# achao2013/deep3dmap

Hardware: AMD Instinct MI355X
Metric: rendered Mpix/s fwd+bwd, 100k-tri mesh @512x512 (higher is better)
Workload: dtype f32

## Files before the change

### deep3dmap_amd/csrc/d3m_forward.h

```cpp
#pragma once
#include "d3m_device.h"

namespace d3m {

struct BinBuffers {
    int B, F, S, tiles_x, tiles_y, T, kcap;
    void* rect;
    int* tile_count;
    int* tile_cursor;
    int* big_count;
    int* alloc_cursor;
    int* tile_offset;
    int* big_list;
    int* pairs;
};

constexpr uint32_t RECT_NONE = 0xFFFFFFFFu;
struct TileRect { int tx0, ty0, w, h; bool none, big; };
struct Rect64 {
    typedef uint2 T;
    static __device__ __forceinline__ T pack(int tx0, int ty0, int tx1, int ty1, bool big) {
        (void)big;
        return make_uint2((uint32_t)tx0 | ((uint32_t)ty0 << 16), (uint32_t)tx1 | ((uint32_t)ty1 << 16));
    }
    static __device__ __forceinline__ T none() { return make_uint2(RECT_NONE, 0); }
    static __device__ __forceinline__ TileRect unpack(T r, int kcap) {
        TileRect t;
        t.none = r.x == RECT_NONE;
        t.tx0 = r.x & 0xFFFF; t.ty0 = r.x >> 16;
        t.w = (int)(r.y & 0xFFFF) - t.tx0 + 1; t.h = (int)(r.y >> 16) - t.ty0 + 1;
        t.big = !t.none && t.w * t.h > kcap;
        return t;
    }
};
struct Rect32 {
    typedef uint32_t T;
    static constexpr uint32_t BIG = 0xFFFFFFFEu;
    static __device__ __forceinline__ T pack(int tx0, int ty0, int tx1, int ty1, bool big) {
        if (big) return BIG;
        return (uint32_t)tx0 | ((uint32_t)ty0 << 10) | ((uint32_t)(tx1 - tx0) << 20) | ((uint32_t)(ty1 - ty0) << 26);
    }
    static __device__ __forceinline__ T none() { return RECT_NONE; }
    static __device__ __forceinline__ TileRect unpack(T r, int kcap) {
        (void)kcap;
        TileRect t;
        t.none = r == RECT_NONE; t.big = r == BIG;
        t.tx0 = r & 0x3FF; t.ty0 = (r >> 10) & 0x3FF; t.w = (int)((r >> 20) & 0x3F) + 1; t.h = (int)(r >> 26) + 1;
        return t;
    }
};

__device__ __forceinline__ bool pixel_bbox(const float* f, int S, int& x0, int& x1, int& y0, int& y1) {
    if (f[0] == f[3] && f[3] == f[6] && f[1] == f[4] && f[4] == f[7]) return false;
    const bool finite = __builtin_isfinite(f[0]) && __builtin_isfinite(f[1]) && __builtin_isfinite(f[3]) &&
                        __builtin_isfinite(f[4]) && __builtin_isfinite(f[6]) && __builtin_isfinite(f[7]);
    if (!finite) {
        x0 = 0; y0 = 0; x1 = S - 1; y1 = S - 1;
        return true;
    }
    const float xmn = fminf(f[0], fminf(f[3], f[6])), xmx = fmaxf(f[0], fmaxf(f[3], f[6]));
    const float ymn = fminf(f[1], fminf(f[4], f[7])), ymx = fmaxf(f[1], fmaxf(f[4], f[7]));
    const double m = 4e-6 * ((double)fmaxf(fmaxf(fabsf(xmn), fabsf(xmx)), fmaxf(fabsf(ymn), fabsf(ymx))) + 1.0);
    const double lx = ceil((((double)xmn - m) * S + S - 1) * 0.5), hx = floor((((double)xmx + m) * S + S - 1) * 0.5);
    const double ly = ceil((((double)ymn - m) * S + S - 1) * 0.5), hy = floor((((double)ymx + m) * S + S - 1) * 0.5);
    if (lx > S - 1 || hx < 0 || ly > S - 1 || hy < 0 || lx > hx || ly > hy) return false;
    x0 = d2i(fmax(lx, 0.0));
    y0 = d2i(fmax(ly, 0.0));
    x1 = d2i(fmin(hx, (double)(S - 1)));
    y1 = d2i(fmin(hy, (double)(S - 1)));
    return true;
}

#ifndef D3M_BIN_THREADS
#define D3M_BIN_THREADS 1024
#endif
constexpr int BIN_THREADS = D3M_BIN_THREADS;
constexpr int BIN_THREADS_SMALL = 256;
constexpr int TA_BITS = BIN_THREADS >= 1024 ? 11 : BIN_THREADS >= 512 ? 10 : 9;
constexpr int TA_SLOTS = 1 << TA_BITS;
constexpr int TA_PROBES = 12;
constexpr int BIN_TABLE_TILES = 4;
__device__ __forceinline__ int ta_bits() { return blockDim.x >= 1024 ? TA_BITS : blockDim.x >= 512 ? TA_BITS - 1 : TA_BITS - 2; }
struct TileAgg {
    int key[TA_SLOTS];
    int cnt[TA_SLOTS];
    int base[TA_SLOTS];
};

__device__ __forceinline__ void ta_clear(TileAgg& t) {
    for (int k = threadIdx.x; k < (1 << ta_bits()); k += blockDim.x) { t.key[k] = 0; t.cnt[k] = 0; }
    __syncthreads();
}

__device__ __forceinline__ int ta_add(TileAgg& t, int tile, int& rank) {
    const int bits = ta_bits();
    unsigned h = ((unsigned)tile * 2654435761u) >> (32 - bits);
    for (int p = 0; p < TA_PROBES; p++, h = (h + 1) & ((1u << bits) - 1)) {
        int k = t.key[h];
        if (k == 0) k = atomicCAS(&t.key[h], 0, tile + 1);
        if (k == 0 || k == tile + 1) {
            rank = atomicAdd(&t.cnt[h], 1);
            return (int)h;
        }
    }
    return -1;
}

template <class FS, bool PAIRED, class RECT>
__global__ void __launch_bounds__(BIN_THREADS) k_bin_count(FS fs, BinBuffers bb, float* __restrict__ faces_inv,
                                                  float* __restrict__ faces_dense_out,
                                                  unsigned char* __restrict__ marks = nullptr,
                                                  int* __restrict__ marks_count = nullptr) {
    __shared__ TileAgg agg;
    if (marks_count && blockIdx.x == 0 && threadIdx.x == 0) *marks_count = 0;
    ta_clear(agg);
    const int F = bb.F, Fl = PAIRED ? F / 2 : F;
    const long lane_i = (long)blockIdx.x * blockDim.x + threadIdx.x;
    const bool in_range = lane_i < (long)bb.B * Fl;
    const int b = in_range ? (int)(lane_i / Fl) : 0, f0 = in_range ? (int)(lane_i % Fl) : 0;
    float loaded[9] = {0, 0, 0, 0, 0, 0, 0, 0, 0};
    if (in_range) fs.load(b, f0, loaded);
#pragma unroll
    for (int side = 0; side < (PAIRED ? 2 : 1); side++) {
        const int f = f0 + side * Fl;
        const long i = (long)b * F + f;
        float face[9];
#pragma unroll
        for (int k = 0; k < 9; k++) face[k] = side == 0 ? loaded[k] : loaded[(2 - k / 3) * 3 + k % 3];
        typename RECT::T r = RECT::none();
        int tx0 = 0, tx1 = -1, ty0 = 0, ty1 = -1;
        bool small = false;
        if (in_range) {
            if (!backside(face)) {
                if (faces_inv) {
                    float fi[9];
                    face_inverse(face, bb.S, fi);
#pragma unroll
                    for (int k = 0; k < 9; k++) faces_inv[i * 9 + k] = fi[k];
                }
                int x0, x1, y0, y1;
                if (pixel_bbox(face, bb.S, x0, x1, y0, y1)) {
                    if (faces_dense_out) {
#pragma unroll
                        for (int k = 0; k < 9; k++) faces_dense_out[i * 9 + k] = face[k];
                    }
                    tx0 = x0 / TILE_W; tx1 = x1 / TILE_W; ty0 = y0 / TILE_H; ty1 = y1 / TILE_H;
                    small = (tx1 - tx0 + 1) * (ty1 - ty0 + 1) <= bb.kcap;
                    r = RECT::pack(tx0, ty0, tx1, ty1, !small);
                    if (!small) {
                        const int pos = atomicAdd(&bb.big_count[b], 1);
                        bb.big_list[(size_t)b * F + pos] = f;
                    }
                }
            }
            reinterpret_cast<typename RECT::T*>(bb.rect)[i] = r;
            if (marks) marks[i] = 0;
        }
        const int w = small ? tx1 - tx0 + 1 : 0, nt = small ? w * (ty1 - ty0 + 1) : 0;
        for (int s = 0; s < nt; s++) {
            const int tile = b * bb.T + (ty0 + s / w) * bb.tiles_x + tx0 + s % w;
            int rank;
            if (s >= BIN_TABLE_TILES || ta_add(agg, tile, rank) < 0) atomicAdd(&bb.tile_count[tile], 1);
        }
    }
    __syncthreads();
    for (int k = threadIdx.x; k < (1 << ta_bits()); k += blockDim.x)
        if (agg.key[k]) atomicAdd(&bb.tile_count[agg.key[k] - 1], agg.cnt[k]);
}

constexpr int BIN_ALLOC_THREADS = 1024;
__global__ void __launch_bounds__(BIN_ALLOC_THREADS) k_bin_alloc(BinBuffers bb) {
    __shared__ int s_wave[BIN_ALLOC_THREADS / 64];
    __shared__ int s_base;
    const int n = bb.B * bb.T;
    const int i = blockIdx.x * BIN_ALLOC_THREADS + threadIdx.x;
    const int c = i < n ? bb.tile_count[i] : 0;
    const int incl = wave_inclusive_scan(c);
    const int lane = lane_id(), wv = threadIdx.x >> 6;
    if (lane == 63) s_wave[wv] = incl;
    __syncthreads();
    if (threadIdx.x == 0) {
        int run = 0;
        for (int k = 0; k < BIN_ALLOC_THREADS / 64; k++) { const int tk = s_wave[k]; s_wave[k] = run; run += tk; }
        s_base = atomicAdd(bb.alloc_cursor, run);
    }
    __syncthreads();
    if (i < n) bb.tile_offset[i] = s_base + s_wave[wv] + incl - c;
}

template <bool PAIRED, int FPT, class RECT>
__global__ void __launch_bounds__(BIN_THREADS) k_bin_fill(BinBuffers bb) {
    const typename RECT::T* __restrict__ rects = reinterpret_cast<const typename RECT::T*>(bb.rect);
    __shared__ TileAgg agg;
    ta_clear(agg);
    const int Fl = PAIRED ? bb.F / 2 : bb.F;
    constexpr int TA_LOCAL = BIN_TABLE_TILES;
    int packed[FPT][TA_LOCAL], face_of[FPT];
#pragma unroll
    for (int it = 0; it < FPT; it++) {
        const long lane_i = ((long)blockIdx.x * FPT + it) * blockDim.x + threadIdx.x;
        int tx0 = 0, ty0 = 0, w = 0, nt = 0, b = 0, f = 0;
        if (lane_i < (long)bb.B * Fl) {
            b = (int)(lane_i / Fl);
            const int f0 = (int)(lane_i % Fl);
            TileRect r = RECT::unpack(rects[(size_t)b * bb.F + f0], bb.kcap);
            f = f0;
            if (PAIRED) {
                const TileRect r1 = RECT::unpack(rects[(size_t)b * bb.F + f0 + Fl], bb.kcap);
                if (r.none) { r = r1; f = f0 + Fl; }
                else if (!r1.none && !r1.big) {
                    const int an = r1.w * r1.h;
                    for (int s2 = 0; s2 < an; s2++) {
                        const int tile = b * bb.T + (r1.ty0 + s2 / r1.w) * bb.tiles_x + r1.tx0 + s2 % r1.w;
                        const int pos = atomicAdd(&bb.tile_cursor[tile], 1);
                        bb.pairs[(size_t)bb.tile_offset[tile] + pos] = f0 + Fl;
                    }
                }
            }
            if (!r.none && !r.big) {
                tx0 = r.tx0; ty0 = r.ty0;
                w = r.w;
                nt = w * r.h;
            }
        }
        face_of[it] = f;
#pragma unroll
        for (int s = 0; s < TA_LOCAL; s++) packed[it][s] = -1;
        for (int s = 0; s < nt && s < TA_LOCAL; s++) {
            const int tile = b * bb.T + (ty0 + s / w) * bb.tiles_x + tx0 + s % w;
            int rank = 0;
            const int slot = ta_add(agg, tile, rank);
            if (slot >= 0) {
#pragma unroll
                for (int q = 0; q < TA_LOCAL; q++) if (q == s) packed[it][q] = (slot << 16) | rank;
            } else {
                const int pos = atomicAdd(&bb.tile_cursor[tile], 1);
                bb.pairs[(size_t)bb.tile_offset[tile] + pos] = f;
            }
        }
        for (int s0 = TA_LOCAL; s0 < nt; s0 += 4) {
            int tile[4], pos[4], off[4];
#pragma unroll
            for (int j = 0; j < 4; j++) {
                const int s = min(s0 + j, nt - 1);
                tile[j] = b * bb.T + (ty0 + s / w) * bb.tiles_x + tx0 + s % w;
            }
#pragma unroll
            for (int j = 0; j < 4; j++) {
                if (s0 + j < nt) { pos[j] = atomicAdd(&bb.tile_cursor[tile[j]], 1); off[j] = bb.tile_offset[tile[j]]; }
            }
#pragma unroll
            for (int j = 0; j < 4; j++)
                if (s0 + j < nt) bb.pairs[(size_t)off[j] + pos[j]] = f;
        }
    }
    __syncthreads();
    for (int k = threadIdx.x; k < (1 << ta_bits()); k += blockDim.x)
        if (agg.key[k]) {
            const int tile = agg.key[k] - 1;
            agg.base[k] = bb.tile_offset[tile] + atomicAdd(&bb.tile_cursor[tile], agg.cnt[k]);
        }
    __syncthreads();
#pragma unroll
    for (int it = 0; it < FPT; it++) {
#pragma unroll
        for (int s = 0; s < TA_LOCAL; s++)
            if (packed[it][s] >= 0) bb.pairs[(size_t)agg.base[packed[it][s] >> 16] + (packed[it][s] & 0xFFFF)] = face_of[it];
    }
}

__device__ __forceinline__ void wave_lds_sync() {
    __builtin_amdgcn_fence(__ATOMIC_RELEASE, "wavefront");
    __builtin_amdgcn_wave_barrier();
    __builtin_amdgcn_fence(__ATOMIC_ACQUIRE, "wavefront");
}

struct ModeOut {
    float* alpha_map = nullptr;
    float* alpha_out = nullptr;
    float* depth_out = nullptr;
    __device__ __forceinline__ void write(size_t i, size_t o, bool covered, float depth) const {
        const float a = covered ? 1.0f : 0.0f;
        if (alpha_map) alpha_map[i] = a;
        if (alpha_out) alpha_out[o] = a;
        if (depth_out) depth_out[o] = depth;
    }
};
struct RasterOut {
    int32_t* face_index_map;
    float* weight_map;
    float* depth_map;
    float* face_inv_map;
    unsigned char* marks;
    int* marks_count = nullptr;
};

#ifndef D3M_RT_STREAM_WAVES
#define D3M_RT_STREAM_WAVES 5
#endif
template <class FS, int W, bool STREAM = false, bool MODE = false>
__global__ void __launch_bounds__(64 * W, STREAM ? D3M_RT_STREAM_WAVES : 1) k_raster_tiles(FS fs, BinBuffers bb, RasterOut out, float near, float far,
                                                                                          ModeOut mo) {
    static_assert(!STREAM || W == 1, "the streaming form is the one-wave form");
    __shared__ float s_face_all[W][9][WAVE];
    __shared__ float s_finv_all[W][9][WAVE];
    __shared__ int s_fid_all[W][WAVE];
    __shared__ uint32_t s_box_all[W][WAVE];
    __shared__ uint32_t s_zkey_all[W][WAVE];
    __shared__ int s_pre_all[W][WAVE + 1];
    constexpr int RING = 2 * WAVE;
    __shared__ unsigned short s_ring_all[W][RING];
    constexpr int HEADS = 8 * WAVE;
    __shared__ __attribute__((aligned(16))) unsigned char s_head_all[W][HEADS];
    __shared__ unsigned long long s_z[TILE_PX];
    __shared__ float s_cx[TILE_W], s_cy[TILE_H];
    const int wv = W == 1 ? 0 : (int)(threadIdx.x >> 6);
    float (&s_face)[9][WAVE] = s_face_all[wv];
    float (&s_finv)[9][WAVE] = s_finv_all[wv];
    int (&s_fid)[WAVE] = s_fid_all[wv];
    uint32_t (&s_box)[WAVE] = s_box_all[wv];
    uint32_t (&s_zkey)[WAVE] = s_zkey_all[wv];
    int (&s_pre)[WAVE + 1] = s_pre_all[wv];
    unsigned short (&s_ring)[RING] = s_ring_all[wv];
    unsigned char (&s_head)[HEADS] = s_head_all[wv];

    const int n_tiles = bb.B * bb.T;
    const int per = (n_tiles + 7) >> 3;
    const int S = bb.S;
    const int lane = lane_id();
    const int xcd = (int)(blockIdx.x & 7);
    const int tile_stride = STREAM ? (int)(gridDim.x >> 3) : 0;
    const int tile_end = STREAM ? min((xcd + 1) * per, n_tiles) : n_tiles;
    int tile = xcd * per + (int)(blockIdx.x >> 3);
    auto next_tile = [&](int from) { return from + tile_stride; };
    if (tile >= tile_end) return;
    int cnt_cur = 0, off_cur = 0, fid_cur = -1, tile_n = 0, cnt_n = 0, off_n = 0;
    float face_held[9] = {0, 0, 0, 0, 0, 0, 0, 0, 0};
    if (STREAM) {
        cnt_cur = bb.tile_count[tile]; off_cur = bb.tile_offset[tile];
        if (lane < cnt_cur) { fid_cur = bb.pairs[off_cur + lane]; fs.load(tile / bb.T, fid_cur, face_held); }
        tile_n = next_tile(tile);
        if (tile_n < tile_end) { cnt_n = bb.tile_count[tile_n]; off_n = bb.tile_offset[tile_n]; }
    }
  for (;;) {
    int fid_n = -1, tile_nn = 0, cnt_nn = 0, off_nn = 0;
    bool next_requested = !STREAM;
    if (STREAM) {
        if (lane < cnt_n) fid_n = bb.pairs[off_n + lane];
        tile_nn = next_tile(tile_n);
        if (tile_nn < tile_end) { cnt_nn = bb.tile_count[tile_nn]; off_nn = bb.tile_offset[tile_nn]; }
    }
    const int b = tile / bb.T, t = tile % bb.T;
    const int px0 = (t % bb.tiles_x) * TILE_W, py0 = (t / bb.tiles_x) * TILE_H;

    if (wv == 0) {
        if (lane < TILE_W) s_cx[lane] = pixel_center(px0 + lane, S);
        else if (lane < TILE_W + TILE_H) s_cy[lane - TILE_W] = pixel_center(py0 + lane - TILE_W, S);
#pragma unroll
        for (int h = 0; h < TILE_PX / WAVE; h++) s_z[h * WAVE + lane] = ~0ull;
    }
    if (lane == 0) s_pre[0] = 0;
    if (STREAM) wave_lds_sync(); else __syncthreads();

    for (int which = 0; which < 2; which++) {
        const int* list = which == 0 ? bb.pairs + (STREAM ? off_cur : bb.tile_offset[tile]) : bb.big_list + (size_t)b * bb.F;
        const int n = which == 0 ? (STREAM ? cnt_cur : bb.tile_count[tile]) : bb.big_count[b];
        for (int base = wv * WAVE; base < n; base += W * WAVE) {
            int cnt = 0;
            if (base + lane < n) {
                const bool held = STREAM && which == 0 && base == 0;
                const int fid = held ? fid_cur : list[base + lane];
                float face[9];
                if (held) {
#pragma unroll
                    for (int k = 0; k < 9; k++) face[k] = face_held[k];
                } else {
                    fs.load(b, fid, face);
                }
                int x0, x1, y0, y1;
                if (pixel_bbox(face, S, x0, x1, y0, y1)) {
                    x0 = max(x0, px0); x1 = min(x1, px0 + TILE_W - 1);
                    y0 = max(y0, py0); y1 = min(y1, py0 + TILE_H - 1);
                    if (x0 <= x1 && y0 <= y1) {
                        const int bw = x1 - x0 + 1, bh = y1 - y0 + 1;
                        cnt = bw * bh;
                        float finv[9];
                        face_inverse(face, S, finv);
#pragma unroll
                        for (int k = 0; k < 9; k++) { s_face[k][lane] = face[k]; s_finv[k][lane] = finv[k]; }
                        s_fid[lane] = fid;
                        const float zmin = fminf(face[2], fminf(face[5], face[8]));
                        s_zkey[lane] = (zmin > 0.0f) ? ordered_bits(zmin * 0.99999f) : 0u;
                        s_box[lane] = (uint32_t)(x0 - px0) | ((uint32_t)(y0 - py0) << 4) | ((uint32_t)(bw - 1) << 8) |
                                      ((uint32_t)((65536 + bw - 1) / bw) << 12);
                    }
                }
            }
            if (!next_requested) {
                next_requested = true;
                if (fid_n >= 0) fs.load(tile_n / bb.T, fid_n, face_held);
            }
            const int incl = wave_inclusive_scan(cnt);
            s_pre[lane + 1] = incl;
            const int total = __shfl(incl, 63, 64);
            wave_lds_sync();
            int head = 0, count = 0;
            auto resolve = [&](int n) {
                if (lane < n) {
                    const uint32_t ent = s_ring[(head + lane) & (RING - 1)];
                    const int lo = (int)(ent & 63), lx = (int)((ent >> 6) & 15), ly = (int)(ent >> 10);
                    float face[9], finv[9], w[3], zp;
#pragma unroll
                    for (int k = 0; k < 9; k++) { face[k] = s_face[k][lo]; finv[k] = s_finv[k][lo]; }
                    if (weights_depth(face, finv, px0 + lx, py0 + ly, near, far, w, zp)) {
                        const unsigned long long key = ((unsigned long long)ordered_bits(zp) << 32) | (uint32_t)s_fid[lo];
                        atomicMin(&s_z[ly * TILE_W + lx], key);
                    }
                }
            };
            int carry = 0;
            for (int w0 = 0; w0 < total; w0 += HEADS) {
                reinterpret_cast<uint2*>(s_head)[lane] = make_uint2(0, 0);
                wave_lds_sync();
                const int start = incl - cnt;
                if (cnt > 0 && start >= w0 && start < w0 + HEADS) s_head[start - w0] = (unsigned char)(lane + 1);
                wave_lds_sync();
                const int wend = min(total, w0 + HEADS);
                for (int c0 = w0; c0 < wend; c0 += WAVE) {
                    const int c = c0 + lane;
                    uint32_t own = wave_max_scan(c < wend ? (uint32_t)s_head[c - w0] : 0u);
                    own = max(own, (uint32_t)carry);
                    carry = __builtin_amdgcn_readlane((int)own, 63);
                    bool pass = false;
                    uint32_t ent = 0;
                    if (c < wend) {
                        const int lo = (int)own - 1;
                        const int local = c - s_pre[lo];
                        const uint32_t box = s_box[lo];
                        const int bw = (int)((box >> 8) & 15) + 1;
                        const int row = (int)(((uint32_t)local * (box >> 12)) >> 16);
                        const int lx = (int)(box & 15) + (local - row * bw), ly = (int)((box >> 4) & 15) + row;
                        if (!(s_zkey[lo] > (uint32_t)(s_z[ly * TILE_W + lx] >> 32))) {
                            float face[9];
#pragma unroll
                            for (int k = 0; k < 9; k++) face[k] = (k % 3 == 2) ? 0.0f : s_face[k][lo];
                            pass = inside_face(face, s_cx[lx], s_cy[ly]);
                            ent = (uint32_t)lo | ((uint32_t)lx << 6) | ((uint32_t)ly << 10);
                        }
                    }
                    const unsigned long long m = __builtin_amdgcn_ballot_w64(pass);
                    if (pass) s_ring[(head + count + mask_rank(m)) & (RING - 1)] = (unsigned short)ent;
                    count += __popcll(m);
                    wave_lds_sync();
                    if (count >= WAVE) {
                        resolve(WAVE);
                        head = (head + WAVE) & (RING - 1);
                        count -= WAVE;
                    }
                }
            }
            if (count > 0) resolve(count);
            wave_lds_sync();
        }
    }
    if (!next_requested && fid_n >= 0) fs.load(tile_n / bb.T, fid_n, face_held);
    if (!STREAM) {
        __syncthreads();
        if (wv != 0) return;
    }

#pragma unroll 1
    for (int part = 0; part < TILE_PX / WAVE; part++) {
    const int in_tile = part * WAVE + lane;
    const unsigned long long key = s_z[in_tile];
    const int xi = px0 + in_tile % TILE_W, yi = py0 + in_tile / TILE_W;
    if (out.marks) {
        const int fid = key != ~0ull ? (int)(uint32_t)(key & 0xFFFFFFFFull) : -1;
        const int left = __shfl(fid, lane - 1, 64), up = __shfl(fid, lane - TILE_W, 64);
        if (fid >= 0 && !((lane % TILE_W) && left == fid) && !(lane >= TILE_W && up == fid)) out.marks[(size_t)b * bb.F + fid] = 1;
    }
    if (xi < S && yi < S) {
        const size_t i = ((size_t)b * S + yi) * S + xi;
        if (key != ~0ull) {
            const int fid = (int)(uint32_t)(key & 0xFFFFFFFFull);
            float face[9], finv[9], w[3], zp;
            fs.load(b, fid, face);
            face_inverse(face, S, finv);
            weights_depth(face, finv, xi, yi, near, far, w, zp);
            out.depth_map[i] = zp;
            out.face_index_map[i] = fid;
            out.weight_map[3 * i + 0] = w[0];
            out.weight_map[3 * i + 1] = w[1];
            out.weight_map[3 * i + 2] = w[2];
            if constexpr (MODE) mo.write(i, ((size_t)b * S + (S - 1 - yi)) * S + xi, true, zp);
            if (!MODE && out.face_inv_map) {
#pragma unroll
                for (int k = 0; k < 9; k++) out.face_inv_map[9 * i + k] = finv[k];
            }
        } else {
            if constexpr (MODE) mo.write(i, ((size_t)b * S + (S - 1 - yi)) * S + xi, false, far);
            out.depth_map[i] = far;
            out.face_index_map[i] = -1;
            out.weight_map[3 * i + 0] = 0.0f;
            out.weight_map[3 * i + 1] = 0.0f;
            out.weight_map[3 * i + 2] = 0.0f;
            if (!MODE && out.face_inv_map) {
#pragma unroll
                for (int k = 0; k < 9; k++) out.face_inv_map[9 * i + k] = 0.0f;
            }
        }
    }    }
    if (!STREAM || tile_n >= tile_end) break;
    tile = tile_n; cnt_cur = cnt_n; off_cur = off_n; fid_cur = fid_n;
    tile_n = tile_nn; cnt_n = cnt_nn; off_n = off_nn;
    wave_lds_sync();
  }
}

__global__ void __launch_bounds__(256) k_texture_sampling(const float* __restrict__ faces, const float* __restrict__ textures,
                                                         const int32_t* __restrict__ face_index_map,
                                                         const float* __restrict__ weight_map,
                                                         const float* __restrict__ depth_map, float* __restrict__ rgb_map,
                                                         int32_t* __restrict__ sampling_index_map,
                                                         float* __restrict__ sampling_weight_map, int B, int F, int S, int ts,
                                                         float eps) {
    const long i = (long)blockIdx.x * blockDim.x + threadIdx.x;
    if (i >= (long)B * S * S) return;
    const int fi = face_index_map[i];
    if (fi < 0) return;
    const int bn = (int)(i / ((long)S * S));
    const float* face = faces + ((size_t)bn * F + fi) * 9;
    const size_t tex_base = ((size_t)bn * F + fi) * ts * ts * ts * 3;
    const size_t tex_total = (size_t)B * F * ts * ts * ts * 3;
    const float depth = depth_map[i];
    float tif[3];
#pragma unroll
    for (int k = 0; k < 3; k++) {
        float t = weight_map[3 * i + k] * (float)(ts - 1) * (depth / face[3 * k + 2]);
        t = fmaxf(t, 0.0f);
        t = fminf(t, (float)(ts - 1) - eps);
        tif[k] = t;
    }
    float px[3] = {0, 0, 0};
#pragma unroll
    for (int pn = 0; pn < 8; pn++) {
        float w = 1;
        int tii[3];
#pragma unroll
        for (int k = 0; k < 3; k++) {
            const int fl = f2i(tif[k]);
            if (((pn >> k) & 1) == 0) { w *= 1 - (tif[k] - (float)fl); tii[k] = fl; }
            else                      { w *= tif[k] - (float)fl;       tii[k] = fl + 1; }
        }
        const int isc = tii[0] * ts * ts + tii[1] * ts + tii[2];
#pragma unroll
        for (int k = 0; k < 3; k++) {
            const size_t ti = tex_base + (size_t)((long)isc * 3 + k);
            px[k] += w * (ti < tex_total ? textures[ti] : 0.0f);
        }
        if (sampling_index_map) sampling_index_map[i * 8 + pn] = isc;
        if (sampling_weight_map) sampling_weight_map[i * 8 + pn] = w;
    }
    rgb_map[3 * i + 0] = px[0];
    rgb_map[3 * i + 1] = px[1];
    rgb_map[3 * i + 2] = px[2];
}

}
```

Before: 6235.

## Trim LDS and registers in streaming raster kernel to raise waves per SIMD

Raises the streaming launch-bound occupancy from 5 to 6 waves. To fit that budget it narrows the prefix array to 16-bit when the kernel runs one wave, halves the head buffer for that case, and uses asm barriers to keep S, the mode pointers and the zero constant in scalar or vector registers. It also replaces the shuffle-based wave scan with a DPP scan plus readlane, computes tile coordinates with unsigned division, and reads left/up neighbour ids for marks from LDS instead of using shuffles. Higher occupancy may bring register spills, and the 16-bit prefix relies on per-batch counts staying small.

New measurement: 6285, median of 6. Within noise of the previous version (+0.8%).

```diff
diff --git a/deep3dmap_amd/csrc/d3m_forward.h b/deep3dmap_amd/csrc/d3m_forward.h
--- a/deep3dmap_amd/csrc/d3m_forward.h
+++ b/deep3dmap_amd/csrc/d3m_forward.h
@@ -295,22 +295,36 @@
     int* marks_count = nullptr;
 };
 
+__device__ __forceinline__ int wave_inclusive_scan_dpp(int v) {
+    v += (int)dpp_u32_or0<0x111, 0xF>((uint32_t)v);
+    v += (int)dpp_u32_or0<0x112, 0xF>((uint32_t)v);
+    v += (int)dpp_u32_or0<0x114, 0xF>((uint32_t)v);
+    v += (int)dpp_u32_or0<0x118, 0xF>((uint32_t)v);
+    v += (int)dpp_u32_or0<0x142, 0xA>((uint32_t)v);
+    v += (int)dpp_u32_or0<0x143, 0xC>((uint32_t)v);
+    return v;
+}
+
+template <bool NARROW> struct RasterPrefix { typedef int T; };
+template <> struct RasterPrefix<true> { typedef unsigned short T; };
+
 #ifndef D3M_RT_STREAM_WAVES
-#define D3M_RT_STREAM_WAVES 5
+#define D3M_RT_STREAM_WAVES 6
 #endif
 template <class FS, int W, bool STREAM = false, bool MODE = false>
 __global__ void __launch_bounds__(64 * W, STREAM ? D3M_RT_STREAM_WAVES : 1) k_raster_tiles(FS fs, BinBuffers bb, RasterOut out, float near, float far,
                                                                                           ModeOut mo) {
     static_assert(!STREAM || W == 1, "the streaming form is the one-wave form");
+    typedef typename RasterPrefix<W == 1 && TILE_PX == 64>::T pre_t;
     __shared__ float s_face_all[W][9][WAVE];
     __shared__ float s_finv_all[W][9][WAVE];
     __shared__ int s_fid_all[W][WAVE];
     __shared__ uint32_t s_box_all[W][WAVE];
     __shared__ uint32_t s_zkey_all[W][WAVE];
-    __shared__ int s_pre_all[W][WAVE + 1];
+    __shared__ pre_t s_pre_all[W][WAVE + 1];
     constexpr int RING = 2 * WAVE;
     __shared__ unsigned short s_ring_all[W][RING];
-    constexpr int HEADS = 8 * WAVE;
+    constexpr int HEADS = (W == 1 ? 4 : 8) * WAVE;
     __shared__ __attribute__((aligned(16))) unsigned char s_head_all[W][HEADS];
     __shared__ unsigned long long s_z[TILE_PX];
     __shared__ float s_cx[TILE_W], s_cy[TILE_H];
@@ -320,7 +334,7 @@
     int (&s_fid)[WAVE] = s_fid_all[wv];
     uint32_t (&s_box)[WAVE] = s_box_all[wv];
     uint32_t (&s_zkey)[WAVE] = s_zkey_all[wv];
-    int (&s_pre)[WAVE + 1] = s_pre_all[wv];
+    pre_t (&s_pre)[WAVE + 1] = s_pre_all[wv];
     unsigned short (&s_ring)[RING] = s_ring_all[wv];
     unsigned char (&s_head)[HEADS] = s_head_all[wv];
 
@@ -350,8 +364,8 @@
         tile_nn = next_tile(tile_n);
         if (tile_nn < tile_end) { cnt_nn = bb.tile_count[tile_nn]; off_nn = bb.tile_offset[tile_nn]; }
     }
-    const int b = tile / bb.T, t = tile % bb.T;
-    const int px0 = (t % bb.tiles_x) * TILE_W, py0 = (t / bb.tiles_x) * TILE_H;
+    const int b = (int)((unsigned)tile / (unsigned)bb.T), t = (int)((unsigned)tile % (unsigned)bb.T);
+    const int px0 = (int)((unsigned)t % (unsigned)bb.tiles_x) * TILE_W, py0 = (int)((unsigned)t / (unsigned)bb.tiles_x) * TILE_H;
 
     if (wv == 0) {
         if (lane < TILE_W) s_cx[lane] = pixel_center(px0 + lane, S);
@@ -367,6 +381,8 @@
         const int n = which == 0 ? (STREAM ? cnt_cur : bb.tile_count[tile]) : bb.big_count[b];
         for (int base = wv * WAVE; base < n; base += W * WAVE) {
             int cnt = 0;
+            int S_st = S;
+            if (STREAM) asm volatile("" : "+s"(S_st));
             if (base + lane < n) {
                 const bool held = STREAM && which == 0 && base == 0;
                 const int fid = held ? fid_cur : list[base + lane];
@@ -378,14 +394,14 @@
                     fs.load(b, fid, face);
                 }
                 int x0, x1, y0, y1;
-                if (pixel_bbox(face, S, x0, x1, y0, y1)) {
+                if (pixel_bbox(face, S_st, x0, x1, y0, y1)) {
                     x0 = max(x0, px0); x1 = min(x1, px0 + TILE_W - 1);
                     y0 = max(y0, py0); y1 = min(y1, py0 + TILE_H - 1);
                     if (x0 <= x1 && y0 <= y1) {
                         const int bw = x1 - x0 + 1, bh = y1 - y0 + 1;
                         cnt = bw * bh;
                         float finv[9];
-                        face_inverse(face, S, finv);
+                        face_inverse(face, S_st, finv);
 #pragma unroll
                         for (int k = 0; k < 9; k++) { s_face[k][lane] = face[k]; s_finv[k][lane] = finv[k]; }
                         s_fid[lane] = fid;
@@ -400,9 +416,9 @@
                 next_requested = true;
                 if (fid_n >= 0) fs.load(tile_n / bb.T, fid_n, face_held);
             }
-            const int incl = wave_inclusive_scan(cnt);
-            s_pre[lane + 1] = incl;
-            const int total = __shfl(incl, 63, 64);
+            const int incl = wave_inclusive_scan_dpp(cnt);
+            s_pre[lane + 1] = (pre_t)incl;
+            const int total = __builtin_amdgcn_readlane(incl, 63);
             wave_lds_sync();
             int head = 0, count = 0;
             auto resolve = [&](int n) {
@@ -420,7 +436,8 @@
             };
             int carry = 0;
             for (int w0 = 0; w0 < total; w0 += HEADS) {
-                reinterpret_cast<uint2*>(s_head)[lane] = make_uint2(0, 0);
+                if constexpr (W == 1) reinterpret_cast<uint32_t*>(s_head)[lane] = 0u;
+                else reinterpret_cast<uint2*>(s_head)[lane] = make_uint2(0, 0);
                 wave_lds_sync();
                 const int start = incl - cnt;
                 if (cnt > 0 && start >= w0 && start < w0 + HEADS) s_head[start - w0] = (unsigned char)(lane + 1);
@@ -435,7 +452,7 @@
                     uint32_t ent = 0;
                     if (c < wend) {
                         const int lo = (int)own - 1;
-                        const int local = c - s_pre[lo];
+                        const int local = c - (int)s_pre[lo];
                         const uint32_t box = s_box[lo];
                         const int bw = (int)((box >> 8) & 15) + 1;
                         const int row = (int)(((uint32_t)local * (box >> 12)) >> 16);
@@ -475,12 +492,19 @@
     const unsigned long long key = s_z[in_tile];
     const int xi = px0 + in_tile % TILE_W, yi = py0 + in_tile / TILE_W;
     if (out.marks) {
-        const int fid = key != ~0ull ? (int)(uint32_t)(key & 0xFFFFFFFFull) : -1;
-        const int left = __shfl(fid, lane - 1, 64), up = __shfl(fid, lane - TILE_W, 64);
-        if (fid >= 0 && !((lane % TILE_W) && left == fid) && !(lane >= TILE_W && up == fid)) out.marks[(size_t)b * bb.F + fid] = 1;
+        const int fid = (int)(uint32_t)key;
+        const int left = (lane % TILE_W) ? (int)(uint32_t)s_z[in_tile - 1] : -1;
+        const int up = lane >= TILE_W ? (int)(uint32_t)s_z[in_tile - TILE_W] : -1;
+        if (fid >= 0 && left != fid && up != fid) out.marks[(size_t)b * bb.F + fid] = 1;
     }
     if (xi < S && yi < S) {
         const size_t i = ((size_t)b * S + yi) * S + xi;
+        ModeOut mw = mo;
+        float zero = 0.0f;
+        if (STREAM) {
+            if constexpr (MODE) asm volatile("" : "+s"(mw.alpha_map), "+s"(mw.alpha_out), "+s"(mw.depth_out));
+            asm volatile("" : "+v"(zero));
+        }
         if (key != ~0ull) {
             const int fid = (int)(uint32_t)(key & 0xFFFFFFFFull);
             float face[9], finv[9], w[3], zp;
@@ -492,18 +516,18 @@
             out.weight_map[3 * i + 0] = w[0];
             out.weight_map[3 * i + 1] = w[1];
             out.weight_map[3 * i + 2] = w[2];
-            if constexpr (MODE) mo.write(i, ((size_t)b * S + (S - 1 - yi)) * S + xi, true, zp);
+            if constexpr (MODE) mw.write(i, ((size_t)b * S + (S - 1 - yi)) * S + xi, true, zp);
             if (!MODE && out.face_inv_map) {
 #pragma unroll
                 for (int k = 0; k < 9; k++) out.face_inv_map[9 * i + k] = finv[k];
             }
         } else {
-            if constexpr (MODE) mo.write(i, ((size_t)b * S + (S - 1 - yi)) * S + xi, false, far);
+            if constexpr (MODE) mw.write(i, ((size_t)b * S + (S - 1 - yi)) * S + xi, false, far);
             out.depth_map[i] = far;
             out.face_index_map[i] = -1;
-            out.weight_map[3 * i + 0] = 0.0f;
-            out.weight_map[3 * i + 1] = 0.0f;
-            out.weight_map[3 * i + 2] = 0.0f;
+            out.weight_map[3 * i + 0] = zero;
+            out.weight_map[3 * i + 1] = zero;
+            out.weight_map[3 * i + 2] = zero;
             if (!MODE && out.face_inv_map) {
 #pragma unroll
                 for (int k = 0; k < 9; k++) out.face_inv_map[9 * i + k] = 0.0f;
```
